# JNP-Solutions/Slacken

Measured on AMD Instinct MI355X. Metric: classify_throughput_150bp_standard224scale, higher is better.
Workload: dtype u64

## Files before the change

slacken_amd/csrc/lane.hip:

```cpp
#include "engine.h"

#include <algorithm>
#include <cstddef>
#include <cstdio>
#include <cstdlib>

namespace slk {

#ifndef SLK_LANE_LW
#define SLK_LANE_LW 4
#endif
constexpr int LW = SLK_LANE_LW;
constexpr int QCAP = 128;
#ifndef SLK_SBLK
#define SLK_SBLK 5
#endif
constexpr int SBLK = SLK_SBLK;
#ifndef SLK_OMAP
#define SLK_OMAP 12
#endif
constexpr int OMAP = SLK_OMAP;
constexpr int OMAP_CNT_BITS = 10;
constexpr uint32_t OMAP_CNT_MASK = (1u << OMAP_CNT_BITS) - 1;

struct __attribute__((aligned(16))) LaneLds {
  uint64_t q_key[QCAP];
  uint32_t q_meta[QCAP];
  uint64_t stash[128];
  uint32_t found[64];
  uint4 sbuf[(SBLK - 1) * 64];
  uint32_t omap[OMAP * 64];
  uint32_t o_flags[64];
  uint64_t rb[64];
  uint16_t q_ord[QCAP];
};

#ifdef SLK_TUNING
#define SLK_TUNE(...) __VA_ARGS__
#define SLK_TUNE_ON(bit) ((dbg & (bit)) != 0)
#else
#define SLK_TUNE(...)
#define SLK_TUNE_ON(bit) false
#endif

#ifndef SLK_PROBE_NT
#define SLK_PROBE_NT 0
#endif
__device__ __forceinline__ ulonglong2 SLK_PROBE_LOAD(const ulonglong2 *p) {
#if SLK_PROBE_NT
  ulonglong2 v;
  v.x = __builtin_nontemporal_load(&p->x);
  v.y = __builtin_nontemporal_load(&p->y);
  return v;
#else
  return *p;
#endif
}

__device__ __forceinline__ void lane_wave_sync() {
  __builtin_amdgcn_fence(__ATOMIC_RELEASE, "wavefront");
  __builtin_amdgcn_wave_barrier();
  __builtin_amdgcn_fence(__ATOMIC_ACQUIRE, "wavefront");
}
__device__ __forceinline__ uint64_t lmin64(uint64_t a, uint64_t b) { return a < b ? a : b; }

template <bool LONG>
__device__ __forceinline__ void fold_hit(LaneLds *L, uint32_t *ocnt, bool in, uint32_t meta, int32_t taxon) {
  if (in && taxon != 0) {
    const int owner = meta & 63;
    const int32_t kmers = (int32_t)((meta >> 7) & 0x1FFF);
    if (meta & 64) atomicAdd(&L->o_flags[owner], 1u);
    uint32_t slot = (uint32_t)(((uint64_t)((uint32_t)taxon * 0x9E3779B1u) * (uint32_t)OMAP) >> 32);
    int p = 0;
    if (LONG) {
      for (; p < OMAP; p++) {
        uint32_t old = atomicCAS(&L->omap[slot * 64 + owner], 0u, (uint32_t)taxon);
        if (old == 0u || old == (uint32_t)taxon) { atomicAdd(&ocnt[slot * 64 + owner], (uint32_t)kmers); break; }
        slot = (slot + 1 == (uint32_t)OMAP) ? 0u : slot + 1;
      }
    } else {
      const uint32_t fresh = ((uint32_t)taxon << OMAP_CNT_BITS) | (uint32_t)kmers;
      for (; p < OMAP; p++) {
        uint32_t old = atomicCAS(&L->omap[slot * 64 + owner], 0u, fresh);
        if (old == 0u) break;
        if ((old >> OMAP_CNT_BITS) == (uint32_t)taxon) { atomicAdd(&L->omap[slot * 64 + owner], (uint32_t)kmers); break; }
        slot = (slot + 1 == (uint32_t)OMAP) ? 0u : slot + 1;
      }
    }
    if (p == OMAP) atomicOr(&L->o_flags[owner], 0x80000000u);
  }
}

constexpr int PG = 64 / LPB;
template <bool HITS, bool LONG>
__device__ __forceinline__ int probe_batch(LaneLds *L, uint32_t *ocnt, const TableView &T, int qhead, int qn, int cnt, int lane, int dbg,
                                           int32_t *hit_meta, int32_t *hit_taxon) {
  const uint64_t NO_TAG = ~0ULL;
  const bool in = lane < cnt;
  const int qi = (qhead + lane) & (QCAP - 1);
  const uint64_t key = L->q_key[qi];
  const uint32_t meta = L->q_meta[qi];
  const uint32_t ord = HITS ? L->q_ord[qi] : 0u;
  const uint64_t h = fmix64(key);
  uint32_t home;
// ... 41 lines not shown
      const uint64_t k_old = L->q_key[qj];
      const uint16_t o_old = HITS ? L->q_ord[qj] : (uint16_t)0;
      const uint64_t R = __ballot(again);
      lane_wave_sync();
      if (again) {
        const int slot = (qhead + qn + requeued + __builtin_amdgcn_mbcnt_hi((uint32_t)(R >> 32), __builtin_amdgcn_mbcnt_lo((uint32_t)R, 0))) & (QCAP - 1);
        L->q_key[slot] = k_old;
        L->q_meta[slot] = m_old + (1u << 20);
        if (HITS) L->q_ord[slot] = o_old;
      }
      requeued += __popcll(R);
    }
  }
  lane_wave_sync();
  const int32_t taxon = (int32_t)L->found[lane];
  if (!SLK_TUNE_ON(2)) fold_hit<LONG>(L, ocnt, in, meta, taxon);
  if (HITS && in) {
    const uint64_t at = L->rb[meta & 63] + ord;
    hit_taxon[at] = ext_taxon(T, taxon);
    hit_meta[at] = pack_meta((int32_t)((meta >> 7) & 0x1FFF), 1, (meta >> 6) & 1);
  }
  lane_wave_sync();
  return requeued;
}

#ifndef SLK_STREAM_NT
#define SLK_STREAM_NT 0
#endif
#ifndef SLK_APPLY_ROWS
#define SLK_APPLY_ROWS 4
#endif
// ... 9 lines not shown
  __builtin_nontemporal_store(v, p);
#else
  *p = v;
#endif
}

__device__ __forceinline__ uint64_t lane_readlane64(uint64_t v, int src) {
  uint32_t lo = __builtin_amdgcn_readlane((uint32_t)v, src), hi = __builtin_amdgcn_readlane((uint32_t)(v >> 32), src);
  return ((uint64_t)hi << 32) | lo;
}
__device__ __forceinline__ uint32_t shard_owner(uint64_t key, uint32_t ns) {
  const uint64_t h = fmix64(key);
  return (ns & (ns - 1)) == 0 ? (uint32_t)(h & (ns - 1)) : (uint32_t)(h % ns);
}
__device__ __forceinline__ uint64_t side_load(const ShardIO &S, uint64_t batch, int lane) {
  const uint64_t i = batch * 64 + (uint64_t)lane;
  return i < S.side_n ? (uint64_t)SLK_STREAM_LOAD(&S.side_keys[i]) : 0;
}
__device__ __forceinline__ void side_probe(LaneLds *L, const TableView &T, const ShardIO &S, int lane, uint64_t batch, uint64_t key, int dbg) {
  const uint64_t base = batch * 64;
  if (base >= S.side_n) return;
  const uint64_t i = base + (uint64_t)lane;
  const bool in = i < S.side_n;
  const uint64_t h = fmix64(key);
  uint32_t home;
  uint64_t rem_hi;
  table_slot(T.g, h, home, rem_hi);
  const uint64_t tag = in ? rem_hi : ~0ULL;
  uint4 st;
  st.x = home; st.y = 0; st.z = (uint32_t)tag; st.w = (uint32_t)(tag >> 32);
  ((uint4 *)L->stash)[lane] = st;
  L->found[lane] = 0;
  lane_wave_sync();
  const int g = lane / LPB, c = lane % LPB;
  const uint64_t tmask = (1ULL << T.g.taxon_bits) - 1;
  const char *cellbase = (const char *)T.cells + c * 16;
// ... 33 lines not shown
        has_empty |= (v.x == 0) | (v.y == 0);
        if (q == 0) closed = T.g.flag != 0 && (v.x & T.g.flag) == 0;
        if (v.x != 0 && cell_tag(T.g, v.x) == want) hit = (int32_t)(v.x & tmask);
        if (v.y != 0 && cell_tag(T.g, v.y) == want) hit = (int32_t)(v.y & tmask);
      }
      if (hit) { taxon = hit; break; }
      if (has_empty || closed) break;
    }
  }
  if (in && !SLK_TUNE_ON(128)) SLK_STREAM_STORE(&S.side_out[i], ext_taxon(T, taxon));
  lane_wave_sync();
}

template <bool HITS>
__device__ __forceinline__ void apply_rows(LaneLds *L, const ApplyJob &J, int lane, uint64_t row0, uint32_t nrows) {
  const uint32_t ns = (uint32_t)J.n_shards;
  constexpr int U = SLK_APPLY_ROWS;
  for (uint32_t b = 0; b < nrows; b += U) {
    uint64_t at[U];
    bool in[U];
#pragma unroll
    for (int u = 0; u < U; u++) {
      in[u] = false;
      at[u] = 0;
      if (b + u < nrows) {
        uint32_t off = 0;
        for (uint32_t sh = 0; sh < ns; sh++) {
          const uint4 e = J.batch_log[(row0 + b + u) * ns + sh];
          const uint32_t cnt = e.z;
          if (cnt == 0) continue;
// ... 7 lines not shown
      }
    }
    uint32_t meta[U];
    int32_t taxon[U];
#pragma unroll
    for (int u = 0; u < U; u++) {
      meta[u] = in[u] ? SLK_STREAM_LOAD(&J.send_meta[at[u]]) : 0u;
      taxon[u] = in[u] ? SLK_STREAM_LOAD(&J.taxa[at[u]]) : 0;
    }
#pragma unroll
    for (int u = 0; u < U; u++) {
      if (b + u < nrows) {
        int32_t t = taxon[u];
        if (in[u]) {
          if (HITS) {
            const uint64_t hat = L->rb[meta[u] & 63] + (meta[u] >> 20);
            J.A.span_taxon[hat] = t;
            J.A.span_meta[hat] = pack_meta((int32_t)((meta[u] >> 7) & 0x1FFF), 1, (meta[u] >> 6) & 1);
          }
          if (J.to_dense != nullptr && t > 0) t = t < J.n_to_dense ? J.to_dense[t] : 0;
        }
        fold_hit<false>(L, nullptr, in[u], meta[u], t);
      }
    }
    lane_wave_sync();
  }
}

template <bool HITS>
__device__ __forceinline__ void emit_batch(LaneLds *L, const FusedArgs &A, const ShardIO &S, const ApplyJob &J, int qhead, int cnt, int lane,
                                           uint64_t row, uint64_t tile, uint32_t &ch_pos, uint32_t &ch_end, uint32_t &side_j, uint64_t &side_key, int dbg) {
  SLK_TUNE(if (dbg & 256) return;)
  const bool in = lane < cnt;
  const int qi = (qhead + lane) & (QCAP - 1);
  const uint64_t key = L->q_key[qi];
  const uint32_t meta = L->q_meta[qi] | (HITS ? (uint32_t)L->q_ord[qi] << 20 : 0u);
  const uint32_t ns = (uint32_t)S.n_shards;
  const uint32_t g = ns == 1 ? 0u : shard_owner(key, ns);
  uint32_t mycount = 0, rank = 0;
  for (uint32_t sh = 0; sh < ns; sh++) {
    const uint64_t m = __ballot(in && g == sh);
    if ((uint32_t)lane == sh) mycount = (uint32_t)__popcll(m);
    if (g == sh) rank = __builtin_amdgcn_mbcnt_hi((uint32_t)(m >> 32), __builtin_amdgcn_mbcnt_lo((uint32_t)m, 0));
  }
  const uint32_t pos = ch_pos, room = ch_end - ch_pos;
  const bool need = (uint32_t)lane < ns && mycount > room;
  unsigned long long got = 0;
  if (need) got = atomicAdd(&S.cursors[lane], (unsigned long long)S.chunk);
  if (side_j < S.side_per_tile) {
    const uint64_t batch = tile * S.side_per_tile + side_j;
    const uint64_t k_now = side_key;
    side_j++;
    if (side_j < S.side_per_tile) side_key = side_load(S, batch + 1, lane);
    side_probe(L, A.T, S, lane, batch, k_now, dbg);
  }
  uint32_t fresh = 0xFFFFFFFFu;
  if (need) {
    if (got + S.chunk <= S.cap) fresh = (uint32_t)got;
    else atomicOr(A.status, 2);
  }
  if ((uint32_t)lane < ns) {
    S.batch_log[row * ns + (uint32_t)lane] = make_uint4(pos, fresh, mycount, room);
    if (need) { ch_pos = fresh == 0xFFFFFFFFu ? 0u : fresh + (mycount - room); ch_end = fresh == 0xFFFFFFFFu ? 0u : fresh + S.chunk; }
    else ch_pos = pos + mycount;
  }
  const uint32_t gpos = (uint32_t)__shfl((int)pos, (int)g), groom = (uint32_t)__shfl((int)room, (int)g), gfresh = (uint32_t)__shfl((int)fresh, (int)g);
  if (in) {
    const bool tail = rank >= groom;
    if ((!tail || gfresh != 0xFFFFFFFFu) && !SLK_TUNE_ON(32)) {
      const uint64_t at = (uint64_t)g * S.cap + (tail ? gfresh + (rank - groom) : gpos + rank);
      SLK_STREAM_STORE(&S.send_keys[at], (int64_t)key);
      SLK_STREAM_STORE(&S.send_meta[at], meta);
    }
  }
  lane_wave_sync();
}

__device__ __forceinline__ uint4 lane_node(const uint4 *nodes, int32_t ntax, int32_t t) {
  return ((uint32_t)t < (uint32_t)ntax) ? nodes[t] : make_uint4(0u, 0x40000000u + (uint32_t)t, 0x40000000u + (uint32_t)t, 0u);
// ... 127 lines not shown
    }
    __syncthreads();
#pragma unroll
    for (int j = 0; j < PER; j++)
      if (route[j] >= 0)
        A.hand_lists[HandOn::list_at(route[j], A.hand_stride, A.hand_long_cap) + base[route[j]] + rank[j]] =
            (uint32_t)(c * chunk + (uint64_t)j * 256 + threadIdx.x);
    __syncthreads();
  }
}
void launch_route(const FusedArgs &A, hipStream_t s) {
  if (A.R == 0) return;
  hipLaunchKernelGGL(route_kernel, dim3((unsigned)std::min<uint64_t>((A.R + 2047) / 2048, 2048)), dim3(256), 0, s, A);
}

template <bool HITS, bool LONG>
__device__ __forceinline__ void resolve_lane(LaneLds *L, uint32_t *ocnt, const FusedArgs &A, int lane, uint64_t r, uint32_t oflags, int32_t total,
                                             int32_t nhits, int32_t np, int dbg) {
  const int32_t nd = (int32_t)oflags;
  uint32_t *const ecnt = LONG ? ocnt : L->omap;
  int D = 0;
  for (int s = 0; s < OMAP; s++) {
    const uint32_t e = L->omap[s * 64 + lane];
    if (e != 0) {
      if (LONG) ocnt[D * 64 + lane] = ocnt[s * 64 + lane];
      L->omap[D * 64 + lane] = e;
      D++;
    }
  }
#define ENT_TAXON(j) (LONG ? (int32_t)L->omap[(j) * 64 + lane] : (int32_t)(L->omap[(j) * 64 + lane] >> OMAP_CNT_BITS))
#define ENT_COUNT(j) (LONG ? (int32_t)ecnt[(j) * 64 + lane] : (int32_t)(ecnt[(j) * 64 + lane] & OMAP_CNT_MASK))
  int32_t maxTaxon = D ? ENT_TAXON(0) : 0;
  const int32_t c0 = D ? ENT_COUNT(0) : 0;
  uint32_t *const tin = (uint32_t *)L, *const tout = tin + OMAP * 64;
  static_assert(offsetof(LaneLds, omap) >= 2 * OMAP * 64 * sizeof(uint32_t), "the intervals alias the queue and the read stream's slots");
  uint32_t m_in = 0, m_out = 0;
  int32_t sum_all = c0;
  if (D >= 2 && !SLK_TUNE_ON(16)) {
#pragma unroll
    for (int j = 0; j < OMAP; j++) {
      if (j < D) {
        const uint4 nj = lane_node(A.nodes, A.ntax, ENT_TAXON(j));
        tin[j * 64 + lane] = nj.y;
        tout[j * 64 + lane] = nj.z;
      }
    }
    maxTaxon = 0;
    sum_all = 0;
    int32_t best = 0;
    for (int a = 0; a < D; a++) {
      const uint32_t ain = tin[a * 64 + lane], aout = tout[a * 64 + lane];
      int32_t score = 0;
      for (int b = 0; b < D; b++)
        score += (tin[b * 64 + lane] <= ain && ain <= tout[b * 64 + lane]) ? ENT_COUNT(b) : 0;
      sum_all += ENT_COUNT(a);
      if (score > best) {
        maxTaxon = ENT_TAXON(a); best = score; m_in = ain; m_out = aout;
      } else if (score == best) {
        if (m_in <= ain && ain <= m_out) {
        } else if (ain <= m_in && m_in <= aout) {
          maxTaxon = ENT_TAXON(a); m_in = ain; m_out = aout;
        } else {
          int32_t x = (int32_t)lane_node(A.nodes, A.ntax, maxTaxon).x;
          uint4 nx = make_uint4(0, 0, 0, 0);
          while (x != 0) {
            nx = lane_node(A.nodes, A.ntax, x);
            if (nx.y <= ain && ain <= nx.z) break;
            x = (int32_t)nx.x;
          }
// ... 6 lines not shown
  for (int32_t c = 0; c < A.C; c++) {
    const double required = ceil(__dmul_rn(A.thr.v[c], (double)total));
    int32_t mt = maxTaxon;
    if (D < 2 || SLK_TUNE_ON(16)) {
      if ((double)c0 < required) mt = 0;
    } else {
      uint32_t cin = m_in, cout = m_out;
      uint4 cur = make_uint4(0, 0, 0, 0);
      bool have_cur = false;
      while (mt != 0) {
        int32_t ms = 0;
        bool side = false;
        int up = -1;
        uint32_t up_in = 0;
        for (int j = 0; j < D; j++) {
          const uint32_t jin = tin[j * 64 + lane], jout = tout[j * 64 + lane];
          const bool inside = cin <= jin && jin <= cout;
          ms += inside ? ENT_COUNT(j) : 0;
          const bool above = !inside && jin <= cin && cin <= jout;
          side = side || (!inside && !above);
          if (above && (up < 0 || jin > up_in)) { up = j; up_in = jin; }
        }
        if ((double)ms >= required) break;
        if (ms == sum_all) { mt = 0; break; }
        if (!side) {
          mt = ENT_TAXON(up); cin = up_in; cout = tout[up * 64 + lane];
          have_cur = false;
        } else {
          if (!have_cur) cur = lane_node(A.nodes, A.ntax, mt);
          mt = (int32_t)cur.x;
          if (mt != 0) { cur = lane_node(A.nodes, A.ntax, mt); have_cur = true; cin = cur.y; cout = cur.z; }
        }
      }
    }
    bool classified = (mt != 0) && (nd >= A.min_hit_groups);
    A.out_taxon[(uint64_t)c * A.out_stride + r] = classified ? ext_taxon(A.T, mt) : 0;
    A.out_classified[(uint64_t)c * A.out_stride + r] = classified ? 1 : 0;
  }
#undef ENT_TAXON
#undef ENT_COUNT
  if (A.out_nd) A.out_nd[r] = nd;
  if (A.out_tk) A.out_tk[r] = total;
  if (A.out_nh) A.out_nh[r] = nhits;
  if (HITS) A.span_count[r] = nhits;
  if (A.out_np) A.out_np[r] = np;
}

template <bool W5, int MODE, bool HITS, bool LONG>
__device__ __forceinline__ void lane_body(const FusedArgs &A, const ShardIO &S, const ApplyJob *Jp, int32_t *defer, uint32_t max_len, int dbg) {
  extern __shared__ __attribute__((aligned(16))) unsigned char lds_raw[];
  const int lane = threadIdx.x & 63;
  const int wib = __builtin_amdgcn_readfirstlane(threadIdx.x >> 6);
  const ScanParams P = A.P;
  const int k = P.k, m = P.m, w = P.w;
  const size_t fixed = HITS ? sizeof(LaneLds) : offsetof(LaneLds, rb);
  const size_t win_bytes = W5 ? 0 : (size_t)w * 64 * sizeof(uint64_t);
  const size_t per_wave = fixed + win_bytes + (LONG ? (size_t)OMAP * 64 * sizeof(uint32_t) : 0);
  LaneLds *L = (LaneLds *)(lds_raw + (size_t)wib * per_wave);
  uint64_t *win = (uint64_t *)((unsigned char *)L + fixed);
  uint32_t *ocnt = LONG ? (uint32_t *)((unsigned char *)L + fixed + win_bytes) : nullptr;
  const bool paired = A.mate_bases != nullptr;
  const bool scans = MODE != LANE_EMIT || A.R != 0;
  const uint64_t bases_end = scans ? A.offsets[A.R] : 0, mates_end = (scans && paired) ? A.mate_offsets[A.R] : 0;
  uint64_t cls_n[5] = {0, 0, 0, 0, 0}, cls_tiles[5] = {0, 0, 0, 0, 0};
  uint64_t ntiles = (A.R + 63) / 64;
  if (LONG) {
    ntiles = 0;
#pragma unroll
    for (int c = 0; c < 5; c++) {
      cls_n[c] = c == 0 ? (A.route_first ? A.hand_hdr[HandOn::N_SHORT] : 0ULL) : A.hand_hdr[c - 1];
      cls_tiles[c] = (cls_n[c] + 63) / 64;
      ntiles += cls_tiles[c];
    }
  }
  const uint64_t nwaves = (uint64_t)gridDim.x * LW;
  const uint64_t etiles = ntiles;
  const uint64_t atiles = MODE == LANE_EMIT ? (Jp->A.R + 63) / 64 : 0;
  if (MODE == LANE_EMIT) ntiles = max(etiles, atiles);
  uint32_t ch_pos = 0, ch_end = 0;

  for (uint64_t tile = (uint64_t)blockIdx.x * LW + wib, it = 0;; it++) {
    if (LONG) {
      if (it) {
        unsigned long long t = 0;
        if (lane == 0) t = atomicAdd(&A.hand_hdr[HandOn::LONG_DRAW], 1ULL);
        tile = nwaves + lane_readlane64(t, 0);
      }
    } else if (MODE == LANE_EMIT) {
      if (it) {
        unsigned long long t = 0;
        if (lane == 0) t = atomicAdd(&S.cursors[S.n_shards], 1ULL);
        tile = nwaves + lane_readlane64(t, 0);
      }
    } else if (it) {
      tile += nwaves;
    }
    if (tile >= ntiles) break;
    uint64_t unit = tile * 64 + lane;
    bool have = unit < A.R;
    uint64_t r = unit;
    if (LONG) {
      uint64_t local = tile;
      int c = 4;
#pragma unroll
      for (int i = 4; i > 0; i--) if (c == i && local >= cls_tiles[i]) { local -= cls_tiles[i]; c = i - 1; }
      unit = local * 64 + lane;
      have = unit < cls_n[c];
      const uint32_t *const cl = A.hand_lists + HandOn::list_at(c == 0 ? (int)HandOn::SHORT : c - 1, A.hand_stride, A.hand_long_cap);
      r = have ? (uint64_t)cl[unit] : 0;
    }
    const uint8_t *seq = A.bases;
    uint32_t n = 0, n2 = 0;
    uint32_t room = 0;
    if (have) {
      uint64_t o = A.offsets[r];
      seq = A.bases + o;
      n = (uint32_t)(A.offsets[r + 1] - o);
      room = clamp_room(bases_end - o);
      SLK_TUNE(if (dbg & 8) { seq = A.bases + A.offsets[r & 1023]; room = clamp_room(bases_end - A.offsets[r & 1023]); })
      if (paired) n2 = (uint32_t)(A.mate_offsets[r + 1] - A.mate_offsets[r]);
    }
    bool too_long = have && ((uint64_t)n + n2 > max_len);
    bool fin = !have || too_long;
    uint64_t row = 0, row0 = 0;
    if (MODE == LANE_EMIT && tile < etiles) row = row0 = (span_region(A.offsets, A.mate_offsets, tile * 64) >> 6) + tile;
    const uint64_t rbase = (HITS && have) ? span_region(A.offsets, A.mate_offsets, r) : 0;
    if (HITS && MODE != LANE_EMIT) L->rb[lane] = rbase;
#pragma unroll
    for (int s = 0; s < OMAP; s++) L->omap[s * 64 + lane] = 0;
    if (LONG) {
#pragma unroll
      for (int s = 0; s < OMAP; s++) ocnt[s * 64 + lane] = 0;
    }
    L->o_flags[lane] = 0;
    if (MODE == LANE_EMIT && tile < atiles) {
      const uint64_t r2 = tile * 64 + lane;
      const bool have2 = r2 < Jp->A.R;
      const uint2 tr = Jp->tile_rows[tile];
      if (HITS) L->rb[lane] = have2 ? span_region(Jp->A.offsets, Jp->A.mate_offsets, r2) : 0;
      lane_wave_sync();
      apply_rows<HITS>(L, *Jp, lane, tr.x, tr.y);
      const bool dfr2 = have2 && (Jp->defer[r2] != 0 || (L->o_flags[lane] & 0x80000000u));
      const uint64_t DM = __ballot(dfr2);
      if (DM != 0 && lane == 0) atomicAdd(Jp->n_deferred, (unsigned long long)__popcll(DM));
      if (have2) {
        if (dfr2) {
          Jp->defer[r2] = 1;
          if (Jp->A.out_nh) Jp->A.out_nh[r2] = 0;
          if (HITS) Jp->A.span_count[r2] = 0;
        } else {
          const int2 ri = Jp->read_info[r2];
          resolve_lane<HITS, false>(L, nullptr, Jp->A, lane, r2, L->o_flags[lane], ri.x, ri.y, 0, dbg);
        }
      }
      lane_wave_sync();
    }
    uint32_t pos = 0;
    int mate = 0;
    uint32_t cur = 0, b1 = 0, b2 = 0, b3 = 0;
    int sb = 1;
    bool packed = false;
    uint32_t s0 = 0;
    uint32_t *const pcodes = (uint32_t *)L->sbuf;
    uint16_t *const pvalid = (uint16_t *)(pcodes + PACK_WORDS);
    constexpr bool CAN_PACK = SLK_PACKED_STREAM && !LONG && MODE == LANE_LOCAL;
    if (CAN_PACK && !paired) {
      const uint64_t t0 = tile * 64, t1 = min(A.R, t0 + 64);
      const uint64_t span_o = A.offsets[t0], span = A.offsets[t1] - span_o;
      if (span <= PACK_MAX_SPAN && __ballot(!fin) != 0) {
        packed = true;
        s0 = have ? (uint32_t)(A.offsets[r] - span_o) : 0;
        const uint8_t *tb = A.bases + span_o;
        const uint32_t troom = clamp_room(bases_end - span_o), sp = (uint32_t)span;
        constexpr int PG0 = (PACK_LOADS + SLK_PACK_ROUNDS - 1) / SLK_PACK_ROUNDS;
#pragma unroll
        for (int j0 = 0; j0 < PACK_LOADS; j0 += PG0) {
          uint4 v[PG0];
#pragma unroll
          for (int j = 0; j < PG0; j++) {
            const uint32_t cb = (uint32_t)(j0 + j) * 1024u + (uint32_t)lane * 16u;
            v[j] = make_uint4(0, 0, 0, 0);
            if (j0 + j < PACK_LOADS && cb < sp) v[j] = load_block16(tb + cb, troom - cb);
          }
#pragma unroll
          for (int j = 0; j < PG0; j++) {
// ... 2 lines not shown
              uint32_t cw, vw;
              pack16(v[j], cw, vw);
              pcodes[cb >> 4] = cw;
              pvalid[cb >> 4] = (uint16_t)vw;
            }
          }
        }
        lane_wave_sync();
      }
    }
    if (!fin && n > 0) {
      if (CAN_PACK && packed) {
        const uint2 pk = packed_take(pcodes, pvalid, s0);
        cur = pk.x; b1 = pk.y;
      } else {
        uint4 v = stream_refill(L, lane, seq, 0, n, room);
        cur = v.x; b1 = v.y; b2 = v.z; b3 = v.w;
      }
    }
    int run_class = 0;
    uint32_t run_len = 0, nvalid = 0;
    uint64_t fwd = 0, rc = 0;
    uint64_t k1 = ~0ULL, p1 = ~0ULL, p2 = ~0ULL, m41 = ~0ULL;
    uint64_t pre = ~0ULL;
    uint64_t cur_val = 0;
    int32_t cur_run = 0;
    bool first = true, have_last = false;
    uint64_t last_key = 0;
    int32_t total = 0, np = 0, nhits = 0;
    uint32_t side_j = (MODE == LANE_EMIT && S.side_n != 0 && tile < etiles) ? 0u : 0xFFFFFFFFu;
    uint64_t side_key = (MODE == LANE_EMIT && S.side_n != 0 && S.side_per_tile != 0 && tile < etiles) ? side_load(S, tile * S.side_per_tile, lane) : 0;
// ... 74 lines not shown
          if (refill && pos < n) {
            const uint2 pk = packed_take(pcodes, pvalid, s0 + pos);
            cur = pk.x; b1 = pk.y;
          }
        }
      } else {
        const bool nextdw = proc && (pos & 3) == 0;
        cur = nextdw ? b1 : (proc ? (cur >> 8) : cur);
        b1 = nextdw ? b2 : b1;
        b2 = nextdw ? b3 : b2;
        if (__ballot(refill) != 0) {
          if (refill) {
            if (pos < n) {
              uint4 v;
              if (sb < SBLK) { v = L->sbuf[(sb - 1) * 64 + lane]; sb++; }
              else { v = stream_refill(L, lane, seq, pos, n, room); sb = 1; }
              cur = v.x; b1 = v.y; b2 = v.z; b3 = v.w;
            }
          }
        }
      }
      const bool at_end = act && is_end;
      if (__ballot(at_end) != 0) {
        if (at_end) {
          if (mate == 0 && paired) {
            if (HITS) {
              const int32_t ordb = ord0 + ((amb_close || emit) ? 1 : 0);
              A.span_meta[rbase + ordb] = pack_meta(-(k - 1), 3, 0);
              A.span_taxon[rbase + ordb] = -2;
            }
            nhits++;
            first = false;
            mate = 1;
            const uint64_t o2 = A.mate_offsets[r];
            seq = A.mate_bases + o2; n = (uint32_t)(A.mate_offsets[r + 1] - o2); room = clamp_room(mates_end - o2); pos = 0;
            if (n > 0) {
              uint4 v = stream_refill(L, lane, seq, 0, n, room);
              sb = 1;
              cur = v.x; b1 = v.y; b2 = v.z; b3 = v.w;
            }
          } else {
            fin = true;
          }
        }
      }
      if (!W5) {
        if (tphase == w - 1) {
          uint64_t sm = ~0ULL;
          for (int j = w - 1; j >= 0; j--) { sm = lmin64(sm, win[j * 64 + lane]); win[j * 64 + lane] = sm; }
          tphase = 0;
        } else {
          tphase++;
        }
      }
      const bool distinct = emit && (first || !(have_last && ekey == last_key));
      last_key = emit ? ekey : last_key;
      have_last = have_last || emit;
      first = first && !emit;
      total += emit ? ekmers : 0;
      np += emit ? 1 : 0;
      nhits += emit ? 1 : 0;
      uint64_t E = __ballot(emit);
      if (E != 0) {
        if (emit) {
          int slot = (qhead + qn + __builtin_amdgcn_mbcnt_hi((uint32_t)(E >> 32), __builtin_amdgcn_mbcnt_lo((uint32_t)E, 0))) & (QCAP - 1);
          L->q_key[slot] = ekey;
          if (HITS) L->q_ord[slot] = (uint16_t)ord0;
          L->q_meta[slot] = (uint32_t)lane | (distinct ? 64u : 0u) | ((uint32_t)ekmers << 7);
        }
        qn += __popcll(E);
        while (qn >= 64) {
          lane_wave_sync();
          int back = 0;
          if (MODE == LANE_EMIT) emit_batch<HITS>(L, A, S, *Jp, qhead, 64, lane, row++, tile, ch_pos, ch_end, side_j, side_key, dbg);
          else if (!SLK_TUNE_ON(1)) back = probe_batch<HITS, LONG>(L, ocnt, A.T, qhead, qn, 64, lane, dbg, A.span_meta, A.span_taxon);
          qhead = (qhead + 64) & (QCAP - 1);
          qn += back - 64;
        }
      }
    }
    while (qn > 0) {
      lane_wave_sync();
      const int cnt = min(qn, 64);
      int back = 0;
      if (MODE == LANE_EMIT) emit_batch<HITS>(L, A, S, *Jp, qhead, cnt, lane, row++, tile, ch_pos, ch_end, side_j, side_key, dbg);
      else if (!SLK_TUNE_ON(1)) back = probe_batch<HITS, LONG>(L, ocnt, A.T, qhead, qn, cnt, lane, dbg, A.span_meta, A.span_taxon);
      qhead = (qhead + cnt) & (QCAP - 1);
      qn += back - cnt;
    }
    lane_wave_sync();
    if (MODE == LANE_EMIT) {
      if (tile < etiles) {
        if (have) S.read_info[r] = make_int2(total, nhits);
        if (lane == 0) S.tile_rows[tile] = make_uint2((uint32_t)row0, (uint32_t)(row - row0));
      }
      while (side_j < S.side_per_tile) {
        const uint64_t batch = tile * S.side_per_tile + side_j;
        const uint64_t k_now = side_key;
        side_j++;
        if (side_j < S.side_per_tile) side_key = side_load(S, batch + 1, lane);
        side_probe(L, A.T, S, lane, batch, k_now, dbg);
      }
    }

    if (MODE == LANE_LOCAL) {
      const uint32_t oflags = have ? L->o_flags[lane] : 0u;
      const bool dfr = have && (too_long || (oflags & 0x80000000u));
      if (__ballot(dfr) != 0)
        hand_on(A.hand_hdr, A.hand_lists, A.hand_stride, A.hand_long_cap, A.long_max, A.long_bound[0], A.long_bound[1], A.long_bound[2],
                A.seg_min_len, A.wave_min, A.wave_ratio_q10, A.offsets, A.mate_offsets, dfr, too_long, r, lane, LONG);
      if (have && !dfr) resolve_lane<HITS, LONG>(L, ocnt, A, lane, r, oflags, total, nhits, np, dbg);
    } else {
      if (have && too_long) defer[r] = 1;
    }
    lane_wave_sync();
  }
  if (MODE == LANE_EMIT) {
    for (uint32_t sh = 0; sh < (uint32_t)S.n_shards; sh++) {
      const uint32_t p0 = __builtin_amdgcn_readlane(ch_pos, sh), p1 = __builtin_amdgcn_readlane(ch_end, sh);
      for (uint32_t i = p0 + (uint32_t)lane; i < p1; i += 64) S.send_keys[(uint64_t)sh * S.cap + i] = 0;
    }
  }
}

template <bool W5, int MODE, bool HITS, bool LONG>
__global__ void LANE_BOUNDS lane_kernel(FusedArgs A, ShardIO S, int32_t *defer, uint32_t max_len, int dbg) {
  lane_body<W5, MODE, HITS, LONG>(A, S, nullptr, defer, max_len, dbg);
}
template <bool W5, bool HITS>
__global__ void LANE_BOUNDS lane_step_kernel(FusedArgs A, ShardIO S, ApplyJob J, int32_t *defer, uint32_t max_len, int dbg) {
  lane_body<W5, LANE_EMIT, HITS, false>(A, S, &J, defer, max_len, dbg);
}

static size_t lane_lds_per_wave(bool hits, bool w5, int w, bool lng) {
  return (hits ? sizeof(LaneLds) : offsetof(LaneLds, rb)) + (w5 ? 0 : (size_t)w * 64 * sizeof(uint64_t)) + (lng ? (size_t)OMAP * 64 * sizeof(uint32_t) : 0);
}

template <bool HITS, bool LONG>
static void launch_lane_mode(const FusedArgs &A, int32_t *defer, uint32_t max_len, hipStream_t s) {
  if (A.R == 0) return;
  const bool w5 = A.P.w == 5;
  const size_t per_wave = lane_lds_per_wave(HITS, w5, A.P.w, LONG);
  static const int extra_lds = getenv("SLK_LANE_EXTRA_LDS") ? atoi(getenv("SLK_LANE_EXTRA_LDS")) : 0;
  size_t lds = per_wave * LW + (size_t)extra_lds;
  uint64_t tiles = (A.R + 63) / 64;
  uint64_t blocks = (tiles + LW - 1) / LW;
  static const int bpc = getenv("SLK_LANE_BLOCKS_PER_CU") ? atoi(getenv("SLK_LANE_BLOCKS_PER_CU")) : 0;
  if (bpc > 0 && blocks > (uint64_t)256 * bpc) blocks = (uint64_t)256 * bpc;
  if (LONG && blocks > 256 * 5) blocks = 256 * 5;
  dim3 g((unsigned)blocks), b(LW * 64);
// ... 14 lines not shown
}

void launch_lane(const FusedArgs &A, int32_t *defer, uint32_t max_len, hipStream_t s) {
  if (A.span_taxon) launch_lane_mode<true, false>(A, defer, max_len, s);
  else launch_lane_mode<false, false>(A, defer, max_len, s);
}
void launch_lane_long(const FusedArgs &A, uint32_t max_len, hipStream_t s) {
  if (A.span_taxon) launch_lane_mode<true, true>(A, nullptr, max_len, s);
  else launch_lane_mode<false, true>(A, nullptr, max_len, s);
}

template <bool W5, bool HITS>
static void launch_step_mode(const FusedArgs &A, const ShardIO &S, const ApplyJob &J, int32_t *defer, uint32_t max_len, hipStream_t s) {
  const uint64_t tiles = std::max((A.R + 63) / 64, (J.A.R + 63) / 64);
  if (tiles == 0) return;
  const size_t lds = lane_lds_per_wave(HITS, W5, A.P.w, false) * LW;
  static int resident[2][2] = {{0, 0}, {0, 0}};
  static int cus = 0;
  if (cus == 0) {
    int dev = 0;
    (void)hipGetDevice(&dev);
    if (hipDeviceGetAttribute(&cus, hipDeviceAttributeMultiprocessorCount, dev) != hipSuccess || cus <= 0) cus = 256;
  }
  int nb = W5 ? resident[1][HITS] : 0;
  if (nb == 0) {
    if (hipOccupancyMaxActiveBlocksPerMultiprocessor(&nb, (const void *)lane_step_kernel<W5, HITS>, LW * 64, lds) != hipSuccess || nb <= 0) nb = 4;
    if (W5) resident[1][HITS] = nb;
  }
  static const int bpc = getenv("SLK_STEP_BLOCKS_PER_CU") ? atoi(getenv("SLK_STEP_BLOCKS_PER_CU")) : 0;
  if (bpc > 0) nb = bpc;
  const uint64_t blocks = std::min<uint64_t>((tiles + LW - 1) / LW, (uint64_t)cus * nb);
#ifdef SLK_TUNING
  static const int dbg = getenv("SLK_DEBUG_ABLATE") ? atoi(getenv("SLK_DEBUG_ABLATE")) : 0;
#else
  const int dbg = 0;
#endif
  hipLaunchKernelGGL((lane_step_kernel<W5, HITS>), dim3((unsigned)blocks), dim3(LW * 64), lds, s, A, S, J, defer, max_len, dbg);
}
void launch_lane_step(const FusedArgs &A, const ShardIO &S, const ApplyJob &J, int32_t *defer, uint32_t max_len, hipStream_t s) {
  const bool hits = A.R ? A.span_taxon != nullptr : J.A.span_taxon != nullptr;
  if (A.P.w == 5) { if (hits) launch_step_mode<true, true>(A, S, J, defer, max_len, s); else launch_step_mode<true, false>(A, S, J, defer, max_len, s); }
  else { if (hits) launch_step_mode<false, true>(A, S, J, defer, max_len, s); else launch_step_mode<false, false>(A, S, J, defer, max_len, s); }
}

}
```

Baseline: 1157.

## Shrink step kernel LDS footprint and raise waves per EU

After: 1153. About the same (-0.3%).

```diff
diff --git a/slacken_amd/csrc/lane.hip b/slacken_amd/csrc/lane.hip
--- a/slacken_amd/csrc/lane.hip
+++ b/slacken_amd/csrc/lane.hip
@@ -35,6 +35,35 @@
   uint16_t q_ord[QCAP];
 };
 
+template <int MODE> struct LdsView {
+  static constexpr bool STEP = MODE == LANE_EMIT;
+  static constexpr size_t OMAP_AT = STEP ? offsetof(LaneLds, sbuf) : offsetof(LaneLds, omap);
+  static constexpr size_t FLAGS_AT = OMAP_AT + sizeof(uint32_t) * OMAP * 64;
+  static constexpr size_t CH_AT = offsetof(LaneLds, omap);
+  static constexpr size_t RB_AT = STEP ? CH_AT + 2 * 64 * sizeof(uint32_t) : offsetof(LaneLds, rb);
+  static constexpr size_t ORD_AT = RB_AT + sizeof(uint64_t) * 64;
+  static constexpr size_t FIXED = RB_AT;
+  static constexpr size_t FIXED_HITS = ORD_AT + sizeof(uint16_t) * QCAP;
+  static constexpr int ROWS_LOW = (int)(OMAP_AT / 256);
+  static constexpr int ROWS_HIGH = STEP ? (int)((CH_AT - FLAGS_AT) / 256) : 0;
+  static constexpr int NIV = STEP ? ((ROWS_LOW + ROWS_HIGH) / 2 < OMAP ? (ROWS_LOW + ROWS_HIGH) / 2 : OMAP) : OMAP;
+  static __device__ __forceinline__ uint32_t *omap(LaneLds *L) { return (uint32_t *)((unsigned char *)L + OMAP_AT); }
+  static __device__ __forceinline__ uint32_t *o_flags(LaneLds *L) { return (uint32_t *)((unsigned char *)L + FLAGS_AT); }
+  static __device__ __forceinline__ uint64_t *rb(LaneLds *L) { return (uint64_t *)((unsigned char *)L + RB_AT); }
+  static __device__ __forceinline__ uint32_t *chunks(LaneLds *L) { return (uint32_t *)((unsigned char *)L + CH_AT); }
+  static __device__ __forceinline__ uint16_t *q_ord(LaneLds *L) { return (uint16_t *)((unsigned char *)L + ORD_AT); }
+  static constexpr __host__ __device__ int iv_row(int i) { return i < ROWS_LOW ? i : i - ROWS_LOW + (int)(FLAGS_AT / 256); }
+};
+static_assert(LdsView<LANE_LOCAL>::OMAP_AT == offsetof(LaneLds, omap) && LdsView<LANE_LOCAL>::FIXED_HITS == sizeof(LaneLds) &&
+              LdsView<LANE_LOCAL>::NIV == OMAP, "the local kernel's layout is LaneLds as declared");
+static_assert(sizeof(uint32_t) * (OMAP + 1) * 64 <= sizeof(LaneLds::sbuf), "the step's map and flags alias the read stream's slots");
+static_assert(LdsView<LANE_EMIT>::FIXED <= 8192 && LdsView<LANE_EMIT>::FIXED_HITS <= 8192, "the step: five waves per SIMD in 160 KiB");
+static_assert(LdsView<LANE_EMIT>::OMAP_AT % 256 == 0 && LdsView<LANE_EMIT>::FLAGS_AT % 256 == 0, "the interval rows are whole rows");
+template <int MODE> __device__ __forceinline__ int lane_here(int lane) {
+  if (MODE == LANE_EMIT) asm volatile("" : "+v"(lane));
+  return lane;
+}
+
 #ifdef SLK_TUNING
 #define SLK_TUNE(...) __VA_ARGS__
 #define SLK_TUNE_ON(bit) ((dbg & (bit)) != 0)
@@ -64,30 +93,31 @@
 }
 __device__ __forceinline__ uint64_t lmin64(uint64_t a, uint64_t b) { return a < b ? a : b; }
 
-template <bool LONG>
+template <int MODE, bool LONG>
 __device__ __forceinline__ void fold_hit(LaneLds *L, uint32_t *ocnt, bool in, uint32_t meta, int32_t taxon) {
+  uint32_t *const omap = LdsView<MODE>::omap(L), *const o_flags = LdsView<MODE>::o_flags(L);
   if (in && taxon != 0) {
     const int owner = meta & 63;
     const int32_t kmers = (int32_t)((meta >> 7) & 0x1FFF);
-    if (meta & 64) atomicAdd(&L->o_flags[owner], 1u);
+    if (meta & 64) atomicAdd(&o_flags[owner], 1u);
     uint32_t slot = (uint32_t)(((uint64_t)((uint32_t)taxon * 0x9E3779B1u) * (uint32_t)OMAP) >> 32);
     int p = 0;
     if (LONG) {
       for (; p < OMAP; p++) {
-        uint32_t old = atomicCAS(&L->omap[slot * 64 + owner], 0u, (uint32_t)taxon);
+        uint32_t old = atomicCAS(&omap[slot * 64 + owner], 0u, (uint32_t)taxon);
         if (old == 0u || old == (uint32_t)taxon) { atomicAdd(&ocnt[slot * 64 + owner], (uint32_t)kmers); break; }
         slot = (slot + 1 == (uint32_t)OMAP) ? 0u : slot + 1;
       }
     } else {
       const uint32_t fresh = ((uint32_t)taxon << OMAP_CNT_BITS) | (uint32_t)kmers;
       for (; p < OMAP; p++) {
-        uint32_t old = atomicCAS(&L->omap[slot * 64 + owner], 0u, fresh);
+        uint32_t old = atomicCAS(&omap[slot * 64 + owner], 0u, fresh);
         if (old == 0u) break;
-        if ((old >> OMAP_CNT_BITS) == (uint32_t)taxon) { atomicAdd(&L->omap[slot * 64 + owner], (uint32_t)kmers); break; }
+        if ((old >> OMAP_CNT_BITS) == (uint32_t)taxon) { atomicAdd(&omap[slot * 64 + owner], (uint32_t)kmers); break; }
         slot = (slot + 1 == (uint32_t)OMAP) ? 0u : slot + 1;
       }
     }
-    if (p == OMAP) atomicOr(&L->o_flags[owner], 0x80000000u);
+    if (p == OMAP) atomicOr(&o_flags[owner], 0x80000000u);
   }
 }
 
@@ -159,7 +189,7 @@
   }
   lane_wave_sync();
   const int32_t taxon = (int32_t)L->found[lane];
-  if (!SLK_TUNE_ON(2)) fold_hit<LONG>(L, ocnt, in, meta, taxon);
+  if (!SLK_TUNE_ON(2)) fold_hit<LANE_LOCAL, LONG>(L, ocnt, in, meta, taxon);
   if (HITS && in) {
     const uint64_t at = L->rb[meta & 63] + ord;
     hit_taxon[at] = ext_taxon(T, taxon);
@@ -199,12 +229,13 @@
   return (ns & (ns - 1)) == 0 ? (uint32_t)(h & (ns - 1)) : (uint32_t)(h % ns);
 }
 __device__ __forceinline__ uint64_t side_load(const ShardIO &S, uint64_t batch, int lane) {
-  const uint64_t i = batch * 64 + (uint64_t)lane;
+  const uint64_t i = batch * 64 + (uint64_t)lane_here<LANE_EMIT>(lane);
   return i < S.side_n ? (uint64_t)SLK_STREAM_LOAD(&S.side_keys[i]) : 0;
 }
 __device__ __forceinline__ void side_probe(LaneLds *L, const TableView &T, const ShardIO &S, int lane, uint64_t batch, uint64_t key, int dbg) {
   const uint64_t base = batch * 64;
   if (base >= S.side_n) return;
+  lane = lane_here<LANE_EMIT>(lane);
   const uint64_t i = base + (uint64_t)lane;
   const bool in = i < S.side_n;
   const uint64_t h = fmix64(key);
@@ -268,6 +299,7 @@
 
 template <bool HITS>
 __device__ __forceinline__ void apply_rows(LaneLds *L, const ApplyJob &J, int lane, uint64_t row0, uint32_t nrows) {
+  lane = lane_here<LANE_EMIT>(lane);
   const uint32_t ns = (uint32_t)J.n_shards;
   constexpr int U = SLK_APPLY_ROWS;
   for (uint32_t b = 0; b < nrows; b += U) {
@@ -305,13 +337,13 @@
         int32_t t = taxon[u];
         if (in[u]) {
           if (HITS) {
-            const uint64_t hat = L->rb[meta[u] & 63] + (meta[u] >> 20);
+            const uint64_t hat = LdsView<LANE_EMIT>::rb(L)[meta[u] & 63] + (meta[u] >> 20);
             J.A.span_taxon[hat] = t;
             J.A.span_meta[hat] = pack_meta((int32_t)((meta[u] >> 7) & 0x1FFF), 1, (meta[u] >> 6) & 1);
           }
           if (J.to_dense != nullptr && t > 0) t = t < J.n_to_dense ? J.to_dense[t] : 0;
         }
-        fold_hit<false>(L, nullptr, in[u], meta[u], t);
+        fold_hit<LANE_EMIT, false>(L, nullptr, in[u], meta[u], t);
       }
     }
     lane_wave_sync();
@@ -320,23 +352,24 @@
 
 template <bool HITS>
 __device__ __forceinline__ void emit_batch(LaneLds *L, const FusedArgs &A, const ShardIO &S, const ApplyJob &J, int qhead, int cnt, int lane,
-                                           uint64_t row, uint64_t tile, uint32_t &ch_pos, uint32_t &ch_end, uint32_t &side_j, uint64_t &side_key, int dbg) {
+                                           uint64_t row, uint64_t tile, uint32_t &side_j, uint64_t &side_key, int dbg) {
   SLK_TUNE(if (dbg & 256) return;)
-  const bool in = lane < cnt;
-  const int qi = (qhead + lane) & (QCAP - 1);
-  const uint64_t key = L->q_key[qi];
-  const uint32_t meta = L->q_meta[qi] | (HITS ? (uint32_t)L->q_ord[qi] << 20 : 0u);
+  lane = lane_here<LANE_EMIT>(lane);
   const uint32_t ns = (uint32_t)S.n_shards;
-  const uint32_t g = ns == 1 ? 0u : shard_owner(key, ns);
-  uint32_t mycount = 0, rank = 0;
-  for (uint32_t sh = 0; sh < ns; sh++) {
-    const uint64_t m = __ballot(in && g == sh);
-    if ((uint32_t)lane == sh) mycount = (uint32_t)__popcll(m);
-    if (g == sh) rank = __builtin_amdgcn_mbcnt_hi((uint32_t)(m >> 32), __builtin_amdgcn_mbcnt_lo((uint32_t)m, 0));
-  }
-  const uint32_t pos = ch_pos, room = ch_end - ch_pos;
+  uint32_t mycount = 0;
+  {
+    const uint64_t key = L->q_key[(qhead + lane) & (QCAP - 1)];
+    const uint32_t g = ns == 1 ? 0u : shard_owner(key, ns);
+    for (uint32_t sh = 0; sh < ns; sh++) {
+      const uint64_t m = __ballot(lane < cnt && g == sh);
+      if ((uint32_t)lane == sh) mycount = (uint32_t)__popcll(m);
+    }
+  }
+  uint32_t *const ch = LdsView<LANE_EMIT>::chunks(L);
+  const uint32_t pos = ch[lane], room = ch[64 + lane] - pos;
   const bool need = (uint32_t)lane < ns && mycount > room;
   unsigned long long got = 0;
+  asm volatile("" : "+v"(got));
   if (need) got = atomicAdd(&S.cursors[lane], (unsigned long long)S.chunk);
   if (side_j < S.side_per_tile) {
     const uint64_t batch = tile * S.side_per_tile + side_j;
@@ -345,6 +378,17 @@
     if (side_j < S.side_per_tile) side_key = side_load(S, batch + 1, lane);
     side_probe(L, A.T, S, lane, batch, k_now, dbg);
   }
+  lane = lane_here<LANE_EMIT>(lane);
+  const bool in = lane < cnt;
+  const int qi = (qhead + lane) & (QCAP - 1);
+  const uint64_t key = L->q_key[qi];
+  const uint32_t meta = L->q_meta[qi] | (HITS ? (uint32_t)LdsView<LANE_EMIT>::q_ord(L)[qi] << 20 : 0u);
+  const uint32_t g = ns == 1 ? 0u : shard_owner(key, ns);
+  uint32_t rank = 0;
+  for (uint32_t sh = 0; sh < ns; sh++) {
+    const uint64_t m = __ballot(in && g == sh);
+    if (g == sh) rank = __builtin_amdgcn_mbcnt_hi((uint32_t)(m >> 32), __builtin_amdgcn_mbcnt_lo((uint32_t)m, 0));
+  }
   uint32_t fresh = 0xFFFFFFFFu;
   if (need) {
     if (got + S.chunk <= S.cap) fresh = (uint32_t)got;
@@ -352,8 +396,8 @@
   }
   if ((uint32_t)lane < ns) {
     S.batch_log[row * ns + (uint32_t)lane] = make_uint4(pos, fresh, mycount, room);
-    if (need) { ch_pos = fresh == 0xFFFFFFFFu ? 0u : fresh + (mycount - room); ch_end = fresh == 0xFFFFFFFFu ? 0u : fresh + S.chunk; }
-    else ch_pos = pos + mycount;
+    if (need) { ch[lane] = fresh == 0xFFFFFFFFu ? 0u : fresh + (mycount - room); ch[64 + lane] = fresh == 0xFFFFFFFFu ? 0u : fresh + S.chunk; }
+    else ch[lane] = pos + mycount;
   }
   const uint32_t gpos = (uint32_t)__shfl((int)pos, (int)g), groom = (uint32_t)__shfl((int)room, (int)g), gfresh = (uint32_t)__shfl((int)fresh, (int)g);
   if (in) {
@@ -511,26 +555,37 @@
   hipLaunchKernelGGL(route_kernel, dim3((unsigned)std::min<uint64_t>((A.R + 2047) / 2048, 2048)), dim3(256), 0, s, A);
 }
 
-template <bool HITS, bool LONG>
+template <int MODE, bool HITS, bool LONG>
 __device__ __forceinline__ void resolve_lane(LaneLds *L, uint32_t *ocnt, const FusedArgs &A, int lane, uint64_t r, uint32_t oflags, int32_t total,
                                              int32_t nhits, int32_t np, int dbg) {
   const int32_t nd = (int32_t)oflags;
-  uint32_t *const ecnt = LONG ? ocnt : L->omap;
+  using V = LdsView<MODE>;
+  uint32_t *const omap = V::omap(L);
+  uint32_t *const ecnt = LONG ? ocnt : omap;
   int D = 0;
   for (int s = 0; s < OMAP; s++) {
-    const uint32_t e = L->omap[s * 64 + lane];
+    const uint32_t e = omap[s * 64 + lane];
     if (e != 0) {
       if (LONG) ocnt[D * 64 + lane] = ocnt[s * 64 + lane];
-      L->omap[D * 64 + lane] = e;
+      omap[D * 64 + lane] = e;
       D++;
     }
   }
-#define ENT_TAXON(j) (LONG ? (int32_t)L->omap[(j) * 64 + lane] : (int32_t)(L->omap[(j) * 64 + lane] >> OMAP_CNT_BITS))
+#define ENT_TAXON(j) (LONG ? (int32_t)omap[(j) * 64 + lane] : (int32_t)(omap[(j) * 64 + lane] >> OMAP_CNT_BITS))
 #define ENT_COUNT(j) (LONG ? (int32_t)ecnt[(j) * 64 + lane] : (int32_t)(ecnt[(j) * 64 + lane] & OMAP_CNT_MASK))
   int32_t maxTaxon = D ? ENT_TAXON(0) : 0;
   const int32_t c0 = D ? ENT_COUNT(0) : 0;
-  uint32_t *const tin = (uint32_t *)L, *const tout = tin + OMAP * 64;
-  static_assert(offsetof(LaneLds, omap) >= 2 * OMAP * 64 * sizeof(uint32_t), "the intervals alias the queue and the read stream's slots");
+  uint32_t *const ivw = (uint32_t *)L;
+  static_assert(MODE == LANE_EMIT || offsetof(LaneLds, omap) >= 2 * OMAP * 64 * sizeof(uint32_t), "the intervals alias the queue and the read stream's slots");
+  static_assert(V::iv_row(2 * V::NIV - 1) * 256 + 256 <= (int)(MODE == LANE_EMIT ? V::CH_AT : V::FIXED), "the interval rows lie inside the wave's block");
+  auto iv_in = [&](int j) -> uint32_t {
+    if (V::NIV == OMAP || j < V::NIV) return ivw[V::iv_row(j) * 64 + lane];
+    return lane_node(A.nodes, A.ntax, ENT_TAXON(j)).y;
+  };
+  auto iv_out = [&](int j) -> uint32_t {
+    if (V::NIV == OMAP || j < V::NIV) return ivw[V::iv_row(V::NIV + j) * 64 + lane];
+    return lane_node(A.nodes, A.ntax, ENT_TAXON(j)).z;
+  };
   uint32_t m_in = 0, m_out = 0;
   int32_t sum_all = c0;
   if (D >= 2 && !SLK_TUNE_ON(16)) {
@@ -538,18 +593,20 @@
     for (int j = 0; j < OMAP; j++) {
       if (j < D) {
         const uint4 nj = lane_node(A.nodes, A.ntax, ENT_TAXON(j));
-        tin[j * 64 + lane] = nj.y;
-        tout[j * 64 + lane] = nj.z;
+        if (j < V::NIV) {
+          ivw[V::iv_row(j) * 64 + lane] = nj.y;
+          ivw[V::iv_row(V::NIV + j) * 64 + lane] = nj.z;
+        }
       }
     }
     maxTaxon = 0;
     sum_all = 0;
     int32_t best = 0;
     for (int a = 0; a < D; a++) {
-      const uint32_t ain = tin[a * 64 + lane], aout = tout[a * 64 + lane];
+      const uint32_t ain = iv_in(a), aout = iv_out(a);
       int32_t score = 0;
       for (int b = 0; b < D; b++)
-        score += (tin[b * 64 + lane] <= ain && ain <= tout[b * 64 + lane]) ? ENT_COUNT(b) : 0;
+        score += (iv_in(b) <= ain && ain <= iv_out(b)) ? ENT_COUNT(b) : 0;
       sum_all += ENT_COUNT(a);
       if (score > best) {
         maxTaxon = ENT_TAXON(a); best = score; m_in = ain; m_out = aout;
@@ -586,7 +643,7 @@
         int up = -1;
         uint32_t up_in = 0;
         for (int j = 0; j < D; j++) {
-          const uint32_t jin = tin[j * 64 + lane], jout = tout[j * 64 + lane];
+          const uint32_t jin = iv_in(j), jout = iv_out(j);
           const bool inside = cin <= jin && jin <= cout;
           ms += inside ? ENT_COUNT(j) : 0;
           const bool above = !inside && jin <= cin && cin <= jout;
@@ -596,7 +653,7 @@
         if ((double)ms >= required) break;
         if (ms == sum_all) { mt = 0; break; }
         if (!side) {
-          mt = ENT_TAXON(up); cin = up_in; cout = tout[up * 64 + lane];
+          mt = ENT_TAXON(up); cin = up_in; cout = iv_out(up);
           have_cur = false;
         } else {
           if (!have_cur) cur = lane_node(A.nodes, A.ntax, mt);
@@ -625,7 +682,8 @@
   const int wib = __builtin_amdgcn_readfirstlane(threadIdx.x >> 6);
   const ScanParams P = A.P;
   const int k = P.k, m = P.m, w = P.w;
-  const size_t fixed = HITS ? sizeof(LaneLds) : offsetof(LaneLds, rb);
+  using V = LdsView<MODE>;
+  const size_t fixed = HITS ? V::FIXED_HITS : V::FIXED;
   const size_t win_bytes = W5 ? 0 : (size_t)w * 64 * sizeof(uint64_t);
   const size_t per_wave = fixed + win_bytes + (LONG ? (size_t)OMAP * 64 * sizeof(uint32_t) : 0);
   LaneLds *L = (LaneLds *)(lds_raw + (size_t)wib * per_wave);
@@ -649,7 +707,7 @@
   const uint64_t etiles = ntiles;
   const uint64_t atiles = MODE == LANE_EMIT ? (Jp->A.R + 63) / 64 : 0;
   if (MODE == LANE_EMIT) ntiles = max(etiles, atiles);
-  uint32_t ch_pos = 0, ch_end = 0;
+  if (MODE == LANE_EMIT) { V::chunks(L)[lane] = 0; V::chunks(L)[64 + lane] = 0; }
 
   for (uint64_t tile = (uint64_t)blockIdx.x * LW + wib, it = 0;; it++) {
     if (LONG) {
@@ -667,8 +725,9 @@
     } else if (it) {
       tile += nwaves;
     }
-    if (tile >= ntiles) break;
-    uint64_t unit = tile * 64 + lane;
+    if (MODE == LANE_EMIT ? (uint32_t)tile >= (uint32_t)ntiles : tile >= ntiles) break;
+    const int lane_t = lane_here<MODE>(lane);
+    uint64_t unit = tile * 64 + lane_t;
     bool have = unit < A.R;
     uint64_t r = unit;
     if (LONG) {
@@ -697,22 +756,23 @@
     uint64_t row = 0, row0 = 0;
     if (MODE == LANE_EMIT && tile < etiles) row = row0 = (span_region(A.offsets, A.mate_offsets, tile * 64) >> 6) + tile;
     const uint64_t rbase = (HITS && have) ? span_region(A.offsets, A.mate_offsets, r) : 0;
-    if (HITS && MODE != LANE_EMIT) L->rb[lane] = rbase;
-#pragma unroll
-    for (int s = 0; s < OMAP; s++) L->omap[s * 64 + lane] = 0;
+    if (HITS && MODE != LANE_EMIT) V::rb(L)[lane] = rbase;
+#pragma unroll
+    for (int s = 0; s < OMAP; s++) V::omap(L)[s * 64 + lane_t] = 0;
     if (LONG) {
 #pragma unroll
       for (int s = 0; s < OMAP; s++) ocnt[s * 64 + lane] = 0;
     }
-    L->o_flags[lane] = 0;
+    V::o_flags(L)[lane_t] = 0;
     if (MODE == LANE_EMIT && tile < atiles) {
+      const int lane = lane_here<MODE>(threadIdx.x & 63);
       const uint64_t r2 = tile * 64 + lane;
       const bool have2 = r2 < Jp->A.R;
       const uint2 tr = Jp->tile_rows[tile];
-      if (HITS) L->rb[lane] = have2 ? span_region(Jp->A.offsets, Jp->A.mate_offsets, r2) : 0;
+      if (HITS) V::rb(L)[lane] = have2 ? span_region(Jp->A.offsets, Jp->A.mate_offsets, r2) : 0;
       lane_wave_sync();
       apply_rows<HITS>(L, *Jp, lane, tr.x, tr.y);
-      const bool dfr2 = have2 && (Jp->defer[r2] != 0 || (L->o_flags[lane] & 0x80000000u));
+      const bool dfr2 = have2 && (Jp->defer[r2] != 0 || (V::o_flags(L)[lane] & 0x80000000u));
       const uint64_t DM = __ballot(dfr2);
       if (DM != 0 && lane == 0) atomicAdd(Jp->n_deferred, (unsigned long long)__popcll(DM));
       if (have2) {
@@ -722,7 +782,7 @@
           if (HITS) Jp->A.span_count[r2] = 0;
         } else {
           const int2 ri = Jp->read_info[r2];
-          resolve_lane<HITS, false>(L, nullptr, Jp->A, lane, r2, L->o_flags[lane], ri.x, ri.y, 0, dbg);
+          resolve_lane<LANE_EMIT, HITS, false>(L, nullptr, Jp->A, lane, r2, V::o_flags(L)[lane], ri.x, ri.y, 0, dbg);
         }
       }
       lane_wave_sync();
@@ -735,12 +795,13 @@
     uint32_t s0 = 0;
     uint32_t *const pcodes = (uint32_t *)L->sbuf;
     uint16_t *const pvalid = (uint16_t *)(pcodes + PACK_WORDS);
-    constexpr bool CAN_PACK = SLK_PACKED_STREAM && !LONG && MODE == LANE_LOCAL;
-    if (CAN_PACK && !paired) {
+    constexpr bool CAN_PACK = SLK_PACKED_STREAM && !LONG;
+    if (CAN_PACK && !paired && (MODE != LANE_EMIT || tile < etiles)) {
       const uint64_t t0 = tile * 64, t1 = min(A.R, t0 + 64);
       const uint64_t span_o = A.offsets[t0], span = A.offsets[t1] - span_o;
       if (span <= PACK_MAX_SPAN && __ballot(!fin) != 0) {
         packed = true;
+        const int lane = lane_here<MODE>(threadIdx.x & 63);
         s0 = have ? (uint32_t)(A.offsets[r] - span_o) : 0;
         const uint8_t *tb = A.bases + span_o;
         const uint32_t troom = clamp_room(bases_end - span_o), sp = (uint32_t)span;
@@ -773,7 +834,7 @@
         const uint2 pk = packed_take(pcodes, pvalid, s0);
         cur = pk.x; b1 = pk.y;
       } else {
-        uint4 v = stream_refill(L, lane, seq, 0, n, room);
+        uint4 v = stream_refill(L, lane_here<MODE>(lane), seq, 0, n, room);
         cur = v.x; b1 = v.y; b2 = v.z; b3 = v.w;
       }
     }
@@ -878,7 +939,7 @@
             if (pos < n) {
               uint4 v;
               if (sb < SBLK) { v = L->sbuf[(sb - 1) * 64 + lane]; sb++; }
-              else { v = stream_refill(L, lane, seq, pos, n, room); sb = 1; }
+              else { v = stream_refill(L, lane_here<MODE>(lane), seq, pos, n, room); sb = 1; }
               cur = v.x; b1 = v.y; b2 = v.z; b3 = v.w;
             }
           }
@@ -899,7 +960,7 @@
             const uint64_t o2 = A.mate_offsets[r];
             seq = A.mate_bases + o2; n = (uint32_t)(A.mate_offsets[r + 1] - o2); room = clamp_room(mates_end - o2); pos = 0;
             if (n > 0) {
-              uint4 v = stream_refill(L, lane, seq, 0, n, room);
+              uint4 v = stream_refill(L, lane_here<MODE>(lane), seq, 0, n, room);
               sb = 1;
               cur = v.x; b1 = v.y; b2 = v.z; b3 = v.w;
             }
@@ -929,14 +990,14 @@
         if (emit) {
           int slot = (qhead + qn + __builtin_amdgcn_mbcnt_hi((uint32_t)(E >> 32), __builtin_amdgcn_mbcnt_lo((uint32_t)E, 0))) & (QCAP - 1);
           L->q_key[slot] = ekey;
-          if (HITS) L->q_ord[slot] = (uint16_t)ord0;
+          if (HITS) V::q_ord(L)[slot] = (uint16_t)ord0;
           L->q_meta[slot] = (uint32_t)lane | (distinct ? 64u : 0u) | ((uint32_t)ekmers << 7);
         }
         qn += __popcll(E);
         while (qn >= 64) {
           lane_wave_sync();
           int back = 0;
-          if (MODE == LANE_EMIT) emit_batch<HITS>(L, A, S, *Jp, qhead, 64, lane, row++, tile, ch_pos, ch_end, side_j, side_key, dbg);
+          if (MODE == LANE_EMIT) emit_batch<HITS>(L, A, S, *Jp, qhead, 64, lane, row++, tile, side_j, side_key, dbg);
           else if (!SLK_TUNE_ON(1)) back = probe_batch<HITS, LONG>(L, ocnt, A.T, qhead, qn, 64, lane, dbg, A.span_meta, A.span_taxon);
           qhead = (qhead + 64) & (QCAP - 1);
           qn += back - 64;
@@ -947,7 +1008,7 @@
       lane_wave_sync();
       const int cnt = min(qn, 64);
       int back = 0;
-      if (MODE == LANE_EMIT) emit_batch<HITS>(L, A, S, *Jp, qhead, cnt, lane, row++, tile, ch_pos, ch_end, side_j, side_key, dbg);
+      if (MODE == LANE_EMIT) emit_batch<HITS>(L, A, S, *Jp, qhead, cnt, lane, row++, tile, side_j, side_key, dbg);
       else if (!SLK_TUNE_ON(1)) back = probe_batch<HITS, LONG>(L, ocnt, A.T, qhead, qn, cnt, lane, dbg, A.span_meta, A.span_taxon);
       qhead = (qhead + cnt) & (QCAP - 1);
       qn += back - cnt;
@@ -955,7 +1016,9 @@
     lane_wave_sync();
     if (MODE == LANE_EMIT) {
       if (tile < etiles) {
-        if (have) S.read_info[r] = make_int2(total, nhits);
+        const int lane = lane_here<MODE>(threadIdx.x & 63);
+        const uint64_t r = tile * 64 + lane;
+        if (r < A.R) S.read_info[r] = make_int2(total, nhits);
         if (lane == 0) S.tile_rows[tile] = make_uint2((uint32_t)row0, (uint32_t)(row - row0));
       }
       while (side_j < S.side_per_tile) {
@@ -968,20 +1031,21 @@
     }
 
     if (MODE == LANE_LOCAL) {
-      const uint32_t oflags = have ? L->o_flags[lane] : 0u;
+      const uint32_t oflags = have ? V::o_flags(L)[lane] : 0u;
       const bool dfr = have && (too_long || (oflags & 0x80000000u));
       if (__ballot(dfr) != 0)
         hand_on(A.hand_hdr, A.hand_lists, A.hand_stride, A.hand_long_cap, A.long_max, A.long_bound[0], A.long_bound[1], A.long_bound[2],
                 A.seg_min_len, A.wave_min, A.wave_ratio_q10, A.offsets, A.mate_offsets, dfr, too_long, r, lane, LONG);
-      if (have && !dfr) resolve_lane<HITS, LONG>(L, ocnt, A, lane, r, oflags, total, nhits, np, dbg);
+      if (have && !dfr) resolve_lane<LANE_LOCAL, HITS, LONG>(L, ocnt, A, lane, r, oflags, total, nhits, np, dbg);
     } else {
-      if (have && too_long) defer[r] = 1;
+      const uint64_t r = tile * 64 + lane_here<MODE>(threadIdx.x & 63);
+      if (too_long) defer[r] = 1;
     }
     lane_wave_sync();
   }
   if (MODE == LANE_EMIT) {
     for (uint32_t sh = 0; sh < (uint32_t)S.n_shards; sh++) {
-      const uint32_t p0 = __builtin_amdgcn_readlane(ch_pos, sh), p1 = __builtin_amdgcn_readlane(ch_end, sh);
+      const uint32_t p0 = V::chunks(L)[sh], p1 = V::chunks(L)[64 + sh];
       for (uint32_t i = p0 + (uint32_t)lane; i < p1; i += 64) S.send_keys[(uint64_t)sh * S.cap + i] = 0;
     }
   }
@@ -991,13 +1055,15 @@
 __global__ void LANE_BOUNDS lane_kernel(FusedArgs A, ShardIO S, int32_t *defer, uint32_t max_len, int dbg) {
   lane_body<W5, MODE, HITS, LONG>(A, S, nullptr, defer, max_len, dbg);
 }
+#define STEP_BOUNDS __launch_bounds__(LW * 64) __attribute__((amdgpu_waves_per_eu(HITS ? 4 : 5)))
 template <bool W5, bool HITS>
-__global__ void LANE_BOUNDS lane_step_kernel(FusedArgs A, ShardIO S, ApplyJob J, int32_t *defer, uint32_t max_len, int dbg) {
+__global__ void STEP_BOUNDS lane_step_kernel(FusedArgs A, ShardIO S, ApplyJob J, int32_t *defer, uint32_t max_len, int dbg) {
   lane_body<W5, LANE_EMIT, HITS, false>(A, S, &J, defer, max_len, dbg);
 }
 
-static size_t lane_lds_per_wave(bool hits, bool w5, int w, bool lng) {
-  return (hits ? sizeof(LaneLds) : offsetof(LaneLds, rb)) + (w5 ? 0 : (size_t)w * 64 * sizeof(uint64_t)) + (lng ? (size_t)OMAP * 64 * sizeof(uint32_t) : 0);
+static size_t lane_lds_per_wave(bool hits, bool w5, int w, bool lng, bool step = false) {
+  const size_t fixed = step ? (hits ? LdsView<LANE_EMIT>::FIXED_HITS : LdsView<LANE_EMIT>::FIXED) : (hits ? sizeof(LaneLds) : offsetof(LaneLds, rb));
+  return fixed + (w5 ? 0 : (size_t)w * 64 * sizeof(uint64_t)) + (lng ? (size_t)OMAP * 64 * sizeof(uint32_t) : 0);
 }
 
 template <bool HITS, bool LONG>
@@ -1042,7 +1108,7 @@
 static void launch_step_mode(const FusedArgs &A, const ShardIO &S, const ApplyJob &J, int32_t *defer, uint32_t max_len, hipStream_t s) {
   const uint64_t tiles = std::max((A.R + 63) / 64, (J.A.R + 63) / 64);
   if (tiles == 0) return;
-  const size_t lds = lane_lds_per_wave(HITS, W5, A.P.w, false) * LW;
+  const size_t lds = lane_lds_per_wave(HITS, W5, A.P.w, false, true) * LW;
   static int resident[2][2] = {{0, 0}, {0, 0}};
   static int cus = 0;
   if (cus == 0) {
@@ -1071,4 +1137,16 @@
   else { if (hits) launch_step_mode<false, true>(A, S, J, defer, max_len, s); else launch_step_mode<false, false>(A, S, J, defer, max_len, s); }
 }
 
-}
+int lane_step_lds_per_wave(bool hits) { return (int)lane_lds_per_wave(hits, true, 5, false, true); }
+int lane_step_blocks_per_cu(bool hits) {
+  int nb = 0;
+  const size_t lds = lane_lds_per_wave(hits, true, 5, false, true) * LW;
+  const void *fn = hits ? (const void *)lane_step_kernel<true, true> : (const void *)lane_step_kernel<true, false>;
+  if (hipOccupancyMaxActiveBlocksPerMultiprocessor(&nb, fn, LW * 64, lds) != hipSuccess) return -1;
+  return nb;
+}
+
+}
+
+extern "C" int slk_debug_step_lds_per_wave(int hits) { return slk::lane_step_lds_per_wave(hits != 0); }
+extern "C" int slk_debug_step_blocks_per_cu(int hits) { return slk::lane_step_blocks_per_cu(hits != 0); }
```
